# AE-HYU/monte_carlo_localization

Hardware: AMD Instinct MI355X
Metric: MCL updates/sec (particle*beam/s) (higher is better)
Workload: dtype f64; 1 GPU; 4194304 particles/GPU x 1081 beams, Spielberg_map (2000x2000 @ 0.05796), initial cloud N((0.0, 0.0, 0.0),(0.5 m,0.5 m,0.4 rad)) (tracking regime), action (0.05, 0.0, 0.01), stock sensor/motion params, multinomial resampling, Philox seed 42; the timed updates follow 5 warm-up updates (the particle set has resampled to motion-noise width); particles_total=4194304, beams=1081, parallelism=single GPU

## Files before the change

### include/mcl_hip_engine.h

```cpp
#ifndef MCL_HIP_ENGINE_H
#define MCL_HIP_ENGINE_H

#include <stddef.h>
#include <stdint.h>

#ifdef __cplusplus
extern "C" {
#endif

#define MCL_ABI_VERSION 1

typedef struct mcl_engine mcl_engine_t;

typedef enum {
    MCL_OK = 0,
    MCL_ERR_INVALID_ARG = -1,
    MCL_ERR_NOT_READY = -2,
    MCL_ERR_HIP = -3,
    MCL_ERR_NO_DEVICE = -4,
    MCL_ERR_UNSUPPORTED = -5,
    MCL_ERR_PEER = -6,
    MCL_ERR_TIMEOUT = -7
} mcl_status;

// ... 231 lines not shown
    int32_t reserved;
} mcl_recovery_config_t;
void mcl_default_recovery_config(mcl_recovery_config_t *c);
int mcl_set_recovery(mcl_engine_t *h, const mcl_recovery_config_t *c);
int mcl_get_recovery_state(mcl_engine_t *h, double state[3], int64_t *injected_last);
int mcl_set_recovery_state(mcl_engine_t *h, const double state[2]);
int mcl_host_recovery_step(const mcl_recovery_config_t *c, const double in[2], int32_t reset, double max_logw, double sum_w,
                           double denom, int32_t n_beams, double out[2], double *p_next);
int mcl_set_recovery_proposal(mcl_engine_t *h, int32_t n_components, const double *means ,
                              const double *covs , const double *weights );
int mcl_get_recovery_proposal(const mcl_engine_t *h, int32_t *n_components, uint64_t *thresholds, double *factors);
int mcl_host_recovery_proposal(int32_t n_components, const double *means, const double *covs, const double *weights,
                               uint64_t *thresholds, double *factors);

typedef struct {
    double z_hit, z_rand;
    double sigma_hit_m;
    double max_occ_dist_m;
    int32_t reserved[2];
} mcl_likelihood_field_config_t;
void mcl_default_likelihood_field_config(mcl_likelihood_field_config_t *c);
int mcl_set_likelihood_field(mcl_engine_t *h, const mcl_likelihood_field_config_t *c);
int mcl_get_likelihood_field(mcl_engine_t *h, uint16_t *out, size_t n);
int mcl_get_likelihood_table(mcl_engine_t *h, float *out, size_t n, int32_t *K);
int mcl_host_likelihood_field(const int8_t *data, uint32_t width, uint32_t height, float resolution,
                              const mcl_likelihood_field_config_t *c, uint16_t *out, size_t n);
int mcl_host_likelihood_table(const mcl_config_t *cfg, const mcl_likelihood_field_config_t *c, float resolution, float *out,
                              size_t n, int32_t *K);

typedef enum { MCL_MOTION_REFERENCE = 0, MCL_MOTION_DIFF = 1, MCL_MOTION_OMNI = 2 } mcl_motion_model;
typedef struct {
    int32_t model;
    int32_t reserved;
    double alpha1, alpha2, alpha3, alpha4, alpha5;
    double floor_trans_m, floor_rot_rad;
} mcl_motion_config_t;
void mcl_default_motion_config(mcl_motion_config_t *c);
int mcl_set_motion_model(mcl_engine_t *h, const mcl_motion_config_t *c);
int mcl_get_motion_model(const mcl_engine_t *h, mcl_motion_config_t *out);
int mcl_host_motion_scalars(const mcl_motion_config_t *c, const double action[3], double out[8]);
int mcl_host_motion_sample(const mcl_motion_config_t *c, const double action[3], const double *xyz_colmajor,
                           const double *normals_nx3, int64_t n, double *out_colmajor);
int mcl_init_particles_gaussian(mcl_engine_t *h, const double mean[3], const double cov[9], int64_t n,
                                int64_t first_global_index, int64_t n_total);
int mcl_host_gaussian_factor(const double cov[9], double L[6]);
int mcl_init_particles_mixture(mcl_engine_t *h, int32_t n_components, const double *means, const double *covs, const int64_t *counts,
                               int64_t n, int64_t first_global_index, int64_t n_total);

int mcl_host_sensor_table(const mcl_config_t *cfg, int32_t max_range_px, double *out, size_t n);
int mcl_host_skip_field(const int8_t *data, uint32_t width, uint32_t height, uint8_t *out, size_t n);
int mcl_host_skip_field_dir(const int8_t *data, uint32_t width, uint32_t height, int32_t quadrant, uint8_t *out, size_t n);
#define MCL_WEDGES 16
int mcl_host_skip_field_wedge(const int8_t *data, uint32_t width, uint32_t height, int32_t wedge, uint8_t *out, size_t n);
int mcl_host_sweep_global_layout(uint32_t width, uint32_t height, int32_t max_range_px, int64_t out[6]);

typedef enum {
    MCL_BUF_X = 0, MCL_BUF_Y = 1, MCL_BUF_THETA = 2,
    MCL_BUF_QWEIGHT = 3,
    MCL_BUF_LOGW = 4,
    MCL_BUF_SCALARS = 5
} mcl_buffer_id;
int mcl_device_ptr(mcl_engine_t *h, int32_t which, void **dev_ptr);
int mcl_export_state(mcl_engine_t *h, double *d_x, double *d_y, double *d_theta, uint64_t *d_q);
int mcl_get_scalars(mcl_engine_t *h, double out[8]);
int mcl_get_host_scalars(const mcl_engine_t *h, double out[8]);
int mcl_stage_propagate(mcl_engine_t *h, const double *d_px, const double *d_py, const double *d_pth,
                        const uint64_t *d_cdf, int64_t n_parents, uint64_t q_total,
                        int64_t child_first, int64_t n_children_total,
                        const double action[3], const float *obs, int32_t n_beams);
int mcl_stage_resample(mcl_engine_t *h, const double *d_px, const double *d_py, const double *d_pth,
                       const uint64_t *d_cdf, int64_t n_parents, uint64_t q_total,
                       int64_t child_first, int64_t n_children_total, const double action[3]);
int mcl_export_records(mcl_engine_t *h, void *d_records);
int mcl_stage_resample_records(mcl_engine_t *h, const void *d_records, const uint64_t *d_cdf, int64_t n_parents,
                               uint64_t q_total, int64_t child_first, int64_t n_children_total, const double action[3]);
int mcl_stage_distinct_parents(mcl_engine_t *h, const int32_t *d_parent, int64_t n_children, int64_t n_total,
                               int64_t *d_distinct, int32_t *d_slot, int64_t *count);
int mcl_export_records_at(mcl_engine_t *h, const int64_t *d_index, int64_t count, void *d_out);
int mcl_stage_resample_indices(mcl_engine_t *h, const uint64_t *d_cdf, int64_t n_parents, uint64_t q_total, int64_t child_first,
                               int64_t n_children_total, int32_t *d_parent_idx);
int mcl_stage_motion_records(mcl_engine_t *h, const void *d_records, int64_t n_records, const int32_t *d_record_of_child,
                             int64_t child_first, int64_t n_children_total, const double action[3]);
int mcl_compact_chunk_bytes(int64_t chunk_entries, int64_t *bytes);
int mcl_export_compact(mcl_engine_t *h, void *d_chunk, int64_t chunk_entries);
int mcl_stage_resample_compact(mcl_engine_t *h, const void *d_chunks, int32_t n_shards, int64_t chunk_entries, const int64_t *counts,
                               const uint64_t *totals, int64_t n_per_shard, int32_t self_shard, int64_t child_first, int64_t n_children_total,
                               const double action[3]);
int mcl_stage_rays(mcl_engine_t *h, const float *obs, int32_t n_beams);
int mcl_set_reserved_cus(mcl_engine_t *h, int32_t n_cus);
int mcl_stage_weights(mcl_engine_t *h, double global_max_logw);
int mcl_stage_finish(mcl_engine_t *h, const double global_sums[5]);
int mcl_stage_keep(mcl_engine_t *h, int64_t child_first, int64_t n_children_total, const double action[3]);
int mcl_stream_wait_external(mcl_engine_t *h, void *stream);
int mcl_external_wait_stream(mcl_engine_t *h, void *stream);
int mcl_export_compact_async(mcl_engine_t *h, void *d_chunk, int64_t chunk_entries);
int mcl_stage_resample_compact_async(mcl_engine_t *h, const void *d_chunks, int32_t n_shards, int64_t chunk_entries, const int64_t *counts,
                                     const uint64_t *totals, int64_t n_per_shard, int32_t self_shard, int64_t child_first,
                                     int64_t n_children_total, const double action[3]);
int mcl_stage_rays_async(mcl_engine_t *h, const float *obs, int32_t n_beams, double *d_local_max);
int mcl_stage_weights_async(mcl_engine_t *h, const double *d_global_max, double *d_vec, int32_t n_shards, int32_t self_shard);
int mcl_stage_complete(mcl_engine_t *h, const double global_sums[5], int32_t *redo);
int mcl_comm_available(const char **why);
int mcl_comm_unique_id(unsigned char id[128]);
int mcl_comm_create(mcl_engine_t *h, const unsigned char id[128], int32_t n_ranks, int32_t rank);
int mcl_comm_selftest(mcl_engine_t *h);
int mcl_comm_destroy(mcl_engine_t *h);
// ... 36 lines not shown
```

### monte_carlo_localization_amd/csrc/mcl_engine.hip

```cpp
#include "../../include/mcl_hip_engine.h"

#include <hip/hip_runtime.h>
#include <hip/hip_ext.h>
#include <rocprim/device/device_radix_sort.hpp>

#include <algorithm>
#include <chrono>
#include <cmath>
#include <cstdio>
#include <cstring>
#include <string>
#include <vector>

#include "mcl_engine_internal.h"
#include "mcl_kernels.h"
#include "mcl_host_math.h"
#include "mcl_lfield.h"

static_assert(MCL_WEDGES == mcl::kWedges || MCL_KWEDGES != 16, "include/mcl_hip_engine.h and csrc/mcl_wedge.h disagree");

using namespace mcl_host;

namespace {

// ... 921 lines not shown
    h->grid_host.assign(data, data + (size_t)width * height);
    h->map_epoch++;
    h->Wp = h->W + 1; h->Hp = h->H + 1; h->Wps = (h->Wp + 7) & ~7;
    h->tw_cells = 568;
    { const int S = h->env_qside > 0 ? h->env_qside : 280; h->qside = (S - (P + 2) - 3 >= 32) ? S : 0; }
    h->sweep_global = h->env_sweep_global || !mcl::sweep_window_fits(P);
    h->distg_why_not = nullptr;
    const bool want_wedges = h->qside > 0 || h->sweep_global;
    build_sensor_table(h->cfg, P, h->table);
    const int tw = P + 1;
    std::vector<float> L((size_t)tw * tw);
    const double inv_squash = 1.0 / h->cfg.squash_factor;
    for (int r = 0; r < tw; ++r)
        for (int d = 0; d < tw; ++d) L[(size_t)r * tw + d] = (float)(std::log(h->table[(size_t)d * tw + r]) * inv_squash);
    std::vector<uint8_t> dist;
    build_distance_field(data, h->W, h->H, h->Wp, h->Hp, h->Wps, dist);
    h->have_map = false;
    h->d_grid.drop(); h->d_dist.drop(); h->d_dist4.drop(); h->d_L.drop(); h->d_table.drop();
    for (int q = 0; q < 4; ++q) h->d_distq[q].drop();
    MCL_TRY(h->d_grid.reserve(h, (size_t)h->W * h->H));
    MCL_TRY(h->d_dist.reserve(h, dist.size()));
    MCL_TRY(h->d_L.reserve(h, L.size()));
    MCL_TRY(h->d_table.reserve(h, h->table.size()));
    HIPCHK(h, hipMemcpy(h->d_grid, data, (size_t)h->W * h->H, hipMemcpyHostToDevice));
    HIPCHK(h, hipMemcpy(h->d_dist, dist.data(), dist.size(), hipMemcpyHostToDevice));
    {
        std::vector<uint8_t> d4(dist.size() / 2);
        for (size_t k = 0; k < d4.size(); ++k)
            d4[k] = (uint8_t)(std::min<int>(dist[2 * k], 15) | (std::min<int>(dist[2 * k + 1], 15) << 4));
        MCL_TRY(h->d_dist4.reserve(h, d4.size()));
        HIPCHK(h, hipMemcpy(h->d_dist4, d4.data(), d4.size(), hipMemcpyHostToDevice));
    }
    if (want_wedges) {
        static const int qsx[4] = {1, -1, -1, 1}, qsy[4] = {1, 1, -1, -1};
        std::vector<uint8_t> dq;
        for (int q = 0; q < 4; ++q) {
            build_directional_field(data, h->W, h->H, h->Wp, h->Hp, h->Wps, qsx[q], qsy[q], dq);
            MCL_TRY(h->d_distq[q].reserve(h, dq.size()));
            HIPCHK(h, hipMemcpy(h->d_distq[q], dq.data(), dq.size(), hipMemcpyHostToDevice));
        }
    }
    h->d_distw.drop(); h->d_distg.drop();
    if (want_wedges) {
        const size_t fsz = (size_t)h->Hp * h->Wps, ncell = (size_t)h->Hp * h->Wp;
        DevBuf<int32_t> d_nxt, d_prv;
        DevBuf<mcl::WedgeRow> d_rows;
        std::vector<mcl::WedgeRow> rows(2 * mcl::kWedgeR + 1);
        MCL_TRY(h->d_distw.reserve(h, fsz * mcl::kWedges));
        HIPCHK(h, hipMemsetAsync(h->d_distw, 0, fsz * mcl::kWedges, h->stream));
        MCL_TRY(d_nxt.reserve(h, ncell));
        MCL_TRY(d_prv.reserve(h, ncell));
        MCL_TRY(d_rows.reserve(h, rows.size()));
        hipLaunchKernelGGL(mcl::k_row_tables, dim3((h->Hp + 63) / 64), dim3(64), 0, h->stream, h->d_dist, h->Wp, h->Hp, h->Wps, d_nxt, d_prv);
        int rc_w = MCL_OK;
        for (int k = 0; k < mcl::kWedges && rc_w == MCL_OK; ++k) {
            mcl::wedge_rows(k, rows.data());
            if (hipMemcpyAsync(d_rows, rows.data(), rows.size() * sizeof(mcl::WedgeRow), hipMemcpyHostToDevice, h->stream) != hipSuccess ||
                hipStreamSynchronize(h->stream) != hipSuccess) { rc_w = MCL_ERR_HIP; break; }
            hipLaunchKernelGGL(mcl::k_wedge_field, dim3((h->Wp + 255) / 256, h->Hp), dim3(256), 0, h->stream, d_nxt, d_prv, h->Wp, h->Hp, h->Wps,
                               d_rows, h->d_distw + (size_t)k * fsz);
            if (hipStreamSynchronize(h->stream) != hipSuccess) rc_w = MCL_ERR_HIP;
        }
        if (rc_w != MCL_OK) return fail(h, rc_w, "building the wedge fields failed");
        if (h->sweep_global) {
            const mcl::SweepGlobalLayout gl = mcl::sweep_global_layout(h->Wp, h->Hp, P);
            if (!gl.ok) {
                h->distg_why_not = "k_rays_sweep's global-field form needs the sixteen ringed fields (with their tails) in less than 2^32 bytes and rows / pitch below 2^24: this map is too large for it";
            } else {
                h->distg_pitch = gl.pitch;
                h->distg_stride = gl.stride;
                MCL_TRY(h->d_distg.reserve(h, gl.alloc));
                HIPCHK(h, hipMemsetAsync(h->d_distg, 0xFF, gl.alloc, h->stream));
                for (int k = 0; k < mcl::kWedges; ++k) {
                    const int q = k >> mcl::kWedgeShift;
                    hipLaunchKernelGGL(mcl::k_ring_field, dim3((h->distg_pitch + 255) / 256, h->Hp + 4), dim3(256), 0, h->stream, h->d_distw + (size_t)k * fsz,
                                       h->Wp, h->Hp, h->Wps, h->distg_pitch, (q == 0 || q == 3) ? 1 : 0, (q == 0 || q == 1) ? 1 : 0,
                                       h->d_distg + (size_t)k * h->distg_stride);
                }
                HIPCHK(h, hipGetLastError());
                HIPCHK(h, hipStreamSynchronize(h->stream));
            }
        }
    }
    HIPCHK(h, hipMemcpy(h->d_L, L.data(), L.size() * sizeof(float), hipMemcpyHostToDevice));
    HIPCHK(h, hipMemcpy(h->d_table, h->table.data(), h->table.size() * sizeof(double), hipMemcpyHostToDevice));
    h->d_Lt.drop(); h->d_Ltd.drop(); h->ltd_ready = false;
    {
        std::vector<uint32_t> fr;
        for (size_t i = 0; i < (size_t)h->W * h->H; ++i)
            if (data[i] == 0) fr.push_back((uint32_t)i);
        h->d_free.drop();
        h->n_free = fr.size();
        if (h->n_free) {
            MCL_TRY(h->d_free.reserve(h, fr.size()));
            HIPCHK(h, hipMemcpy(h->d_free, fr.data(), fr.size() * sizeof(uint32_t), hipMemcpyHostToDevice));
        }
    }
    h->have_map = true;
    if (h->kld_on) {
        h->kld_nx = kld_nx; h->kld_ny = kld_ny; h->kld_bits = kld_bits;
        const int rc = kld_alloc(h);
        if (rc) { h->have_map = false; return rc; }
    }
    h->lf_K = -1;
    if (h->lf_on) {
        const int rc = lf_build(h);
        if (rc) { h->have_map = false; return rc; }
    }
    return MCL_OK;
}

int mcl_get_max_range_px(const mcl_engine_t *h, int32_t *out)
// ... 1683 lines not shown
```

### monte_carlo_localization_amd/csrc/mcl_host_math.hip

```cpp
#include "mcl_host_math.h"

#include <algorithm>
#include <cmath>
#include <cstring>

#include "mcl_motion.h"
#include "mcl_refine_core.h"
#include "mcl_wedge.h"

namespace mcl_host {

const char *bad_sensor_fields(const mcl_config_t &c)
{
    const double z[4] = {c.z_hit, c.z_short, c.z_max, c.z_rand};
    for (double v : z)
        if (!std::isfinite(v) || v < 0.0) return "bad config (z_hit, z_short, z_max and z_rand must be finite and >= 0)";
    if (z[0] == 0.0 && z[1] == 0.0 && z[2] == 0.0 && z[3] == 0.0) return "bad config (z_hit, z_short, z_max and z_rand are all 0)";
    if (!std::isfinite(c.sigma_hit) || !(c.sigma_hit > 0.0)) return "bad config (sigma_hit must be finite and > 0)";
    return nullptr;
}

void build_sensor_table(const mcl_config_t &c, int P, std::vector<double> &t)
{
    const int tw = P + 1;
// ... 652 lines not shown
        if (thresholds) thresholds[c] = c == M - 1 ? (1ull << 53) : (uint64_t)std::floor((s / total) * 9007199254740992.0);
        if (factors) {
            double *f = factors + 9 * (size_t)c;
            for (int k = 0; k < 3; ++k) f[k] = means[3 * (size_t)c + k];
            (void)gaussian_factor(covs + 9 * (size_t)c, f + 3);
        }
    }
    return std::string();
}

}

using namespace mcl_host;

extern "C" {

void mcl_default_config(mcl_config_t *c)
{
    if (!c) return;
    std::memset(c, 0, sizeof(*c));
    c->max_particles = 2000;
    c->device = 0;
    c->seed = 0;
    c->max_range_m = 12.0;
    c->z_hit = 0.80; c->z_short = 0.01; c->z_max = 0.07; c->z_rand = 0.12; c->sigma_hit = 8.0;
    c->squash_factor = 2.2;
    c->motion_dispersion_x = 0.05; c->motion_dispersion_y = 0.025; c->motion_dispersion_theta = 0.25;
    c->resample_mode = MCL_RESAMPLE_MULTINOMIAL;
    c->weight_mode = MCL_WEIGHT_LOG;
    c->ray_kernel = MCL_RAYS_AUTO;
}

int mcl_host_sensor_table(const mcl_config_t *cfg, int32_t P, double *out, size_t n)
{
    if (!cfg || !out || P < 1 || n != (size_t)(P + 1) * (P + 1) || bad_sensor_fields(*cfg)) return MCL_ERR_INVALID_ARG;
    std::vector<double> t;
    build_sensor_table(*cfg, P, t);
    std::memcpy(out, t.data(), n * sizeof(double));
    return MCL_OK;
}

int mcl_host_skip_field_dir(const int8_t *data, uint32_t width, uint32_t height, int32_t quadrant, uint8_t *out, size_t n)
{
    if (!data || !out || width == 0 || height == 0 || quadrant < 0 || quadrant > 3 || n != (size_t)(width + 1) * (height + 1))
        return MCL_ERR_INVALID_ARG;
    static const int qsx[4] = {1, -1, -1, 1}, qsy[4] = {1, 1, -1, -1};
    const int Wp = (int)width + 1, Hp = (int)height + 1, Wps = (Wp + 7) & ~7;
    std::vector<uint8_t> d;
    build_directional_field(data, (int)width, (int)height, Wp, Hp, Wps, qsx[quadrant], qsy[quadrant], d);
    for (int y = 0; y < Hp; ++y) std::memcpy(out + (size_t)y * Wp, d.data() + (size_t)y * Wps, Wp);
    return MCL_OK;
}

int mcl_host_skip_field_wedge(const int8_t *data, uint32_t width, uint32_t height, int32_t wedge, uint8_t *out, size_t n)
{
    if (!data || !out || width == 0 || height == 0 || wedge < 0 || wedge >= mcl::kWedges || n != (size_t)(width + 1) * (height + 1))
        return MCL_ERR_INVALID_ARG;
    const int W = (int)width, H = (int)height, Wp = W + 1, Hp = H + 1;
    std::vector<int32_t> nxt((size_t)Wp * Hp), prv((size_t)Wp * Hp);
    for (int y = 0; y < Hp; ++y) {
        auto stop = [&](int x) { return data[(size_t)std::max(y - 1, 0) * W + std::max(x - 1, 0)] > 50; };
        int last = -1;
        for (int x = 0; x < Wp; ++x) { if (stop(x)) last = x; prv[(size_t)y * Wp + x] = last; }
        int next = Wp;
        for (int x = Wp - 1; x >= 0; --x) { if (stop(x)) next = x; nxt[(size_t)y * Wp + x] = next; }
    }
    std::vector<mcl::WedgeRow> rows(2 * mcl::kWedgeR + 1);
    mcl::wedge_rows(wedge, rows.data());
    for (int y = 0; y < Hp; ++y)
        for (int x = 0; x < Wp; ++x) out[(size_t)y * Wp + x] = (uint8_t)mcl::wedge_skip_cell(nxt.data(), prv.data(), Wp, Hp, x, y, rows.data());
    return MCL_OK;
}

int mcl_host_skip_field(const int8_t *data, uint32_t width, uint32_t height, uint8_t *out, size_t n)
{
    if (!data || !out || width == 0 || height == 0 || n != (size_t)(width + 1) * (height + 1)) return MCL_ERR_INVALID_ARG;
    const int Wp = (int)width + 1, Hp = (int)height + 1, Wps = (Wp + 7) & ~7;
    std::vector<uint8_t> d;
    build_distance_field(data, (int)width, (int)height, Wp, Hp, Wps, d);
    for (int y = 0; y < Hp; ++y) std::memcpy(out + (size_t)y * Wp, d.data() + (size_t)y * Wps, Wp);
    return MCL_OK;
}

int mcl_host_sweep_global_layout(uint32_t width, uint32_t height, int32_t max_range_px, int64_t out[6])
{
    if (!out || width == 0 || height == 0 || max_range_px < 1) return MCL_ERR_INVALID_ARG;
    const int Wp = (int)width + 1, Hp = (int)height + 1;
    const mcl::SweepGlobalLayout g = mcl::sweep_global_layout(Wp, Hp, max_range_px);
    out[0] = g.ok ? 1 : 0; out[1] = g.pitch; out[2] = g.rows; out[3] = (int64_t)g.stride; out[4] = (int64_t)g.alloc;
    out[5] = (int64_t)mcl::sweep_global_max_offset(g, Wp, Hp, max_range_px, mcl::kWedges - 1);
    return MCL_OK;
}

void mcl_default_kld_config(mcl_kld_config_t *k)
{
    if (!k) return;
    *k = mcl_kld_config_t{};
    k->min_particles = 256; k->max_particles = 4194304;
    k->err = 0.01; k->z = 2.326;
    k->bin_x_m = 0.5; k->bin_y_m = 0.5;
    k->n_theta_bins = 36; k->round_to = 256; k->shrink_permille = 800;
}

int mcl_host_kld_bins(const double *x, const double *y, const double *th, int64_t n, uint32_t width, uint32_t height,
                      float resolution, double origin_x, double origin_y, const mcl_kld_config_t *k, int64_t *bins)
{
    if (!k || !bins || n < 0 || (n > 0 && (!x || !y || !th)) || width == 0 || height == 0 || !(resolution > 0.0f) ||
        !std::isfinite(resolution) || kld_invalid(k, 0))
        return MCL_ERR_INVALID_ARG;
    int64_t nx = 0, ny = 0;
    uint64_t nbits = 0;
    if (!kld_grid(k, width, height, resolution, nx, ny, nbits)) return MCL_ERR_INVALID_ARG;
    const mcl::KldArgs a = kld_args_of(k, nx, ny, origin_x, origin_y);
    std::vector<uint32_t> b((size_t)n);
    for (int64_t i = 0; i < n; ++i) b[(size_t)i] = mcl::kld_bin(a, x[i], y[i], th[i]);
    std::sort(b.begin(), b.end());
    *bins = (int64_t)(std::unique(b.begin(), b.end()) - b.begin());
    return MCL_OK;
}

int mcl_host_kld_target(const mcl_kld_config_t *k, int64_t bins, int64_t n_current, int64_t *n_next)
{
    if (!k || !n_next || n_current < 0 || n_current >= MCL_MAX_TOTAL_PARTICLES || kld_invalid(k, 0)) return MCL_ERR_INVALID_ARG;
// ... 342 lines not shown
```

### monte_carlo_localization_amd/csrc/mcl_kernels.h

```cpp
#pragma once
#include "mcl_types.h"
#include <type_traits>
#include "mcl_ray_core.h"
#include "mcl_device_math.h"
#include "mcl_wedge.h"
#include "mcl_motion.h"

namespace mcl {

constexpr int kRedBlocks = 1024;
constexpr int kRedThreads = 256;
__device__ __forceinline__ void final_sums_of(const double *__restrict__ part, int nb, double *__restrict__ scalars, double (*sm)[7]);


__device__ __forceinline__ uint64_t wave_incl_scan_u64(uint64_t v, int lane)
{
#pragma unroll
    for (int o = 1; o < 64; o <<= 1) {
        uint64_t t = (uint64_t)__shfl_up((long long)v, o, 64);
        if (lane >= o) v += t;
    }
    return v;
}

// ... 1091 lines not shown
        cnt_l2 = wave_sum_u64(cnt_l2);
        if (lane == 0) {
            if (cnt_exact) atomicAdd(&a.counters[0], cnt_exact);
            if (cnt_off) atomicAdd(&a.counters[1], cnt_off);
            if (cnt_probe) atomicAdd(&a.counters[2], cnt_probe);
            if (cnt_l2) atomicAdd(&a.counters[3], cnt_l2);
        }
    }
}

constexpr int kQLdsBase = 16;

__device__ __forceinline__ void quad_ranges(short4 qr, int q, int B, int &ja, int &jb, int &ja2)
{
    const int st1 = qr.x & 0x3FFF, st2 = qr.y, st3 = qr.z, st4 = qr.w, q0 = ((int)qr.x >> 14) & 3;
    const int r_idx = (q - q0) & 3;
    ja = r_idx == 0 ? 0 : (r_idx == 1 ? st1 : (r_idx == 2 ? st2 : st3));
    jb = r_idx == 0 ? st1 : (r_idx == 1 ? st2 : (r_idx == 2 ? st3 : st4));
    ja2 = r_idx == 0 ? st4 : B;
}


__global__ __launch_bounds__(256) void k_ring_field(const uint8_t *__restrict__ src, int Wp, int Hp, int Wps, int pitch, int sxp, int syp,
                                                   uint8_t *__restrict__ dst)
{
    const int x = blockIdx.x * blockDim.x + threadIdx.x, y = blockIdx.y;
    if (x >= pitch) return;
    const int mx = x - 2, my = y - 2;
    uint8_t v = 0xFF;
    if (mx >= 0 && mx < Wp && my >= 0 && my < Hp) v = src[(size_t)(syp ? my : Hp - 1 - my) * Wps + (sxp ? mx : Wp - 1 - mx)];
    dst[(size_t)y * pitch + x] = v;
}

__global__ void k_row_tables(const uint8_t *__restrict__ dist, int Wp, int Hp, int Wps, int32_t *__restrict__ nxt, int32_t *__restrict__ prv)
{
    const int y = blockIdx.x * blockDim.x + threadIdx.x;
    if (y >= Hp) return;
    const uint8_t *row = dist + (size_t)y * Wps;
    int last = -1;
    for (int x = 0; x < Wp; ++x) { if (row[x] == 0) last = x; prv[(size_t)y * Wp + x] = last; }
    int next = Wp;
    for (int x = Wp - 1; x >= 0; --x) { if (row[x] == 0) next = x; nxt[(size_t)y * Wp + x] = next; }
}

__global__ __launch_bounds__(256) void k_wedge_field(const int32_t *__restrict__ nxt, const int32_t *__restrict__ prv, int Wp, int Hp, int Wps,
                                                    const WedgeRow *__restrict__ rows, uint8_t *__restrict__ out)
{
    const int x = blockIdx.x * blockDim.x + threadIdx.x, y = blockIdx.y;
    if (x >= Wp || y >= Hp) return;
    const int v = wedge_skip_cell(nxt, prv, Wp, Hp, x, y, rows);
    out[(size_t)y * Wps + x] = (uint8_t)(v == 0 ? 255 : (v > 127 ? 127 : v));
}

#ifndef MCL_SORT_KEY_LOG2
#define MCL_SORT_KEY_LOG2 22
#endif
constexpr int kSortKeyLog2 = MCL_SORT_KEY_LOG2;
constexpr uint32_t kSortKeySpace = 1u << kSortKeyLog2;
#ifndef MCL_SORT_MAX_SUB
#define MCL_SORT_MAX_SUB 1
#endif
constexpr int kSortXcds = 8;
constexpr uint32_t kSortBuckets = kSortKeySpace * kSortXcds;
constexpr int kHistTile = 4096;

__device__ __forceinline__ int cell_of(double g, int hi)
{
    int c = (g > -1.0) ? ((g < 1e9) ? (int)floor(g) + 1 : hi) : 0;
    return c < 0 ? 0 : (c > hi ? hi : c);
}

__global__ void k_bbox_init(int *__restrict__ bbox, int play)
{
    const int i = threadIdx.x;
    if (i < 7) bbox[i] = i < 2 ? 0x7fffffff : (i < 4 ? (int)0x80000000 : (i == 6 ? play : 0));
}

__global__ __launch_bounds__(256) void k_cell_bbox(const double4 *__restrict__ pc, int64_t n, int stride, int Wp, int Hp, int *__restrict__ bbox,
                                                  int *__restrict__ tilemark = nullptr, int ntx_abs = 0)
{
    int x0 = 0x7fffffff, y0 = 0x7fffffff, x1 = -1, y1 = -1;
    const int64_t ns = (n + stride - 1) / stride;
    for (int64_t k = (int64_t)blockIdx.x * blockDim.x + threadIdx.x; k < ns; k += (int64_t)gridDim.x * blockDim.x) {
        const double4 c = pc[k * stride];
        const int cx = cell_of(c.z * kSortSub, Wp * kSortSub - 1), cy = cell_of(c.w * kSortSub, Hp * kSortSub - 1);
        x0 = min(x0, cx); y0 = min(y0, cy); x1 = max(x1, cx); y1 = max(y1, cy);
        if (tilemark) tilemark[(cy >> 5) * ntx_abs + (cx >> 5)] = 1;
    }
#pragma unroll
    for (int o = 32; o > 0; o >>= 1) {
        x0 = min(x0, __shfl_xor(x0, o, 64)); y0 = min(y0, __shfl_xor(y0, o, 64));
        x1 = max(x1, __shfl_xor(x1, o, 64)); y1 = max(y1, __shfl_xor(y1, o, 64));
    }
    __shared__ int red[4][4];
    const int w = threadIdx.x >> 6;
    if ((threadIdx.x & 63) == 0) { red[w][0] = x0; red[w][1] = y0; red[w][2] = x1; red[w][3] = y1; }
    __syncthreads();
    if (threadIdx.x == 0) {
        for (int k = 1; k < 4; ++k) { x0 = min(x0, red[k][0]); y0 = min(y0, red[k][1]); x1 = max(x1, red[k][2]); y1 = max(y1, red[k][3]); }
        if (x1 >= 0) { atomicMin(&bbox[0], x0); atomicMin(&bbox[1], y0); atomicMax(&bbox[2], x1); atomicMax(&bbox[3], y1); }
    }
}

constexpr int kSortMaxTiles = 8192;
__global__ __launch_bounds__(1024) void k_tile_compact(int *__restrict__ bbox, int *__restrict__ tilemark, int *__restrict__ tilemap, int ntiles_abs)
{
// ... 876 lines not shown
```

### monte_carlo_localization_amd/csrc/mcl_wedge.h

```cpp
#pragma once
#include <cmath>
#include <cstdint>

#ifdef __HIPCC__
#define MCL_HD __host__ __device__
#else
#define MCL_HD
#endif

namespace mcl {

#ifndef MCL_KWEDGES
#define MCL_KWEDGES 16
#endif
constexpr int kWedges = MCL_KWEDGES;
constexpr int kWedgeShift = kWedges == 8 ? 1 : kWedges == 16 ? 2 : kWedges == 32 ? 3 : 4;
static_assert(kWedges == (4 << kWedgeShift), "kWedges must be 8, 16, 32 or 64");
constexpr int kWedgeR = 255;

struct WedgeRow { int16_t xa, xb; };

inline void wedge_rows(int k, WedgeRow *rows)
{
    const double two_pi = 6.283185307179586476925286766559;
// ... 5 lines not shown
    const int sx = (q == 0 || q == 3) ? 1 : -1, sy = (q == 0 || q == 1) ? 1 : -1;
    for (int oy = -kWedgeR; oy <= kWedgeR; ++oy) {
        int xa = 1, xb = 0;
        bool any = false;
        for (int ox = -kWedgeR; ox <= kWedgeR; ++ox) {
            const bool in = sx * ox >= 0 && sy * oy >= 0 && (n1x * ox + n1y * oy + e1 > 1e-9) && (n2x * ox + n2y * oy + e2 > 1e-9);
            if (in) { if (!any) { xa = ox; any = true; } xb = ox; }
        }
        rows[oy + kWedgeR].xa = (int16_t)xa;
        rows[oy + kWedgeR].xb = (int16_t)xb;
    }
}

MCL_HD inline int wedge_skip_cell(const int32_t *nxt, const int32_t *prv, int Wp, int Hp, int x, int y, const WedgeRow *rows)
{
    if (nxt[(size_t)y * Wp + x] == x) return 0;
    int64_t best = (int64_t)1 << 40;
    for (int d = 0; d <= kWedgeR; ++d) {
        const int64_t gy = d > 1 ? d - 1 : 0;
        if (gy * gy >= best) break;
        for (int sgn = (d == 0 ? 1 : -1); sgn <= 1; sgn += 2) {
            const int oy = sgn * d;
            const WedgeRow r = rows[oy + kWedgeR];
            if (r.xa > r.xb) continue;
            const int yy = y + oy, lo = x + r.xa, hi = x + r.xb;
            const bool row_in = yy >= 0 && yy < Hp;
            int ox = 1 << 20;
            if (r.xa <= 0 && r.xb >= 0) {
                const int xr = row_in ? nxt[(size_t)yy * Wp + x] : x;
                const int xl = row_in ? prv[(size_t)yy * Wp + x] : x;
                if (xr <= hi) ox = xr - x;
                if (xl >= lo && x - xl < ox) ox = x - xl;
            } else if (r.xa > 0) {
                const int xr = (!row_in || lo >= Wp) ? lo : nxt[(size_t)yy * Wp + lo];
                if (xr <= hi) ox = xr - x;
            } else {
                const int xl = (!row_in || hi < 0) ? hi : prv[(size_t)yy * Wp + hi];
                if (xl >= lo) ox = x - xl;
            }
            if (ox < (1 << 20)) {
                const int64_t gx = ox > 1 ? ox - 1 : 0;
                const int64_t g2 = gx * gx + gy * gy;
                if (g2 < best) best = g2;
            }
        }
    }
    if (best >= (int64_t)254 * 254) return 255;
    int64_t rt = (int64_t)sqrt((double)best);
    while (rt * rt > best) --rt;
    while ((rt + 1) * (rt + 1) <= best) ++rt;
    return (int)(rt + 1);
}

struct SweepGlobalLayout { bool ok; int pitch; int rows; size_t stride, alloc; };
inline SweepGlobalLayout sweep_global_layout(int Wp, int Hp, int P)
{
    SweepGlobalLayout g{};
    g.pitch = (Wp + 4 + 63) & ~63;
    const int tail = P + 2 + (P + 4 + g.pitch - 1) / g.pitch;
    g.rows = Hp + 4 + tail;
    g.stride = (size_t)g.rows * (size_t)g.pitch;
    g.alloc = g.stride * (size_t)kWedges;
    g.ok = g.alloc < ((size_t)1 << 32) && g.rows + P < (1 << 24) && g.pitch < (1 << 24) && P >= 1;
    return g;
}
inline size_t sweep_global_max_offset(const SweepGlobalLayout &g, int Wp, int Hp, int P, int k)
{
    return (size_t)k * g.stride + (size_t)(Hp + 4 + P) * (size_t)g.pitch + (size_t)(Wp + 4 + P);
}

}
```

### monte_carlo_localization_amd/engine.py

```python
from __future__ import annotations

import ctypes as C
import os

import numpy as np

_HERE = os.path.dirname(os.path.abspath(__file__))
LIB_PATH = os.environ.get("MCL_LIB") or os.path.join(_HERE, "libmcl_hip_engine.so")

MCL_OK = 0
MCL_ERR_INVALID_ARG = -1
MCL_ERR_NOT_READY = -2
MCL_ERR_PEER = -6
MCL_ERR_TIMEOUT = -7
RESAMPLE_MULTINOMIAL, RESAMPLE_SYSTEMATIC = 0, 1
WEIGHT_LOG, WEIGHT_PRODUCT = 0, 1
RAYS_AUTO, RAYS_MARCH, RAYS_SKIP, RAYS_QUAD, RAYS_CELL, RAYS_SWEEP = 0, 1, 2, 3, 4, 5
BUF_X, BUF_Y, BUF_THETA, BUF_QWEIGHT, BUF_LOGW, BUF_SCALARS = range(6)

EXPORTS = [
    "mcl_abi_version", "mcl_default_config", "mcl_create", "mcl_destroy", "mcl_last_error", "mcl_set_map",
    "mcl_get_max_range_px", "mcl_get_sensor_table", "mcl_set_beam_angles", "mcl_set_particles",
    "mcl_get_particles", "mcl_get_weights", "mcl_sample_particles", "mcl_particle_mean", "mcl_update",
    "mcl_sensor_update", "mcl_expected_pose", "mcl_get_stage_timings", "mcl_get_resample_indices",
    "mcl_get_ray_steps", "mcl_get_log_weights", "mcl_get_counters", "mcl_get_ray_kernel_ms", "mcl_device_ptr",
    "mcl_stage_propagate", "mcl_stage_weights", "mcl_stage_finish", "mcl_scan_weights", "mcl_export_state",
    "mcl_get_scalars", "mcl_host_sensor_table", "mcl_host_skip_field", "mcl_init_particles_pose", "mcl_init_global",
    "mcl_update_scan", "mcl_get_ray_kernel_id", "mcl_host_skip_field_dir", "mcl_host_skip_field_wedge", "mcl_export_records", "mcl_get_effective_sample_size", "mcl_get_host_scalars", "mcl_stage_resample_records", "mcl_stage_resample", "mcl_stage_rays",
    "mcl_set_reserved_cus", "mcl_stage_resample_indices", "mcl_stage_motion_records", "mcl_stage_distinct_parents", "mcl_export_records_at",
    "mcl_group_create", "mcl_group_destroy", "mcl_group_last_error", "mcl_group_size", "mcl_group_engine", "mcl_group_set_map",
    "mcl_group_set_beam_angles", "mcl_group_set_particles", "mcl_group_init_particles_pose", "mcl_group_init_global",
    "mcl_group_update", "mcl_group_expected_pose", "mcl_group_get_particles", "mcl_group_get_weights",
    "mcl_group_get_resample_indices", "mcl_group_get_stage_timings", "mcl_group_exchange_bytes",
    "mcl_set_debug_count_probes", "mcl_set_particles_shard", "mcl_get_compact_list", "mcl_compact_chunk_bytes", "mcl_export_compact",
    "mcl_stage_resample_compact", "mcl_group_exchanged_lists", "mcl_get_ray_steps16", "mcl_get_planned_ray_kernel",
    "mcl_stream_wait_external", "mcl_external_wait_stream", "mcl_export_compact_async", "mcl_stage_resample_compact_async",
    "mcl_stage_rays_async", "mcl_stage_weights_async", "mcl_stage_complete", "mcl_stage_keep",
    "mcl_comm_available", "mcl_comm_unique_id", "mcl_comm_create", "mcl_comm_destroy", "mcl_comm_update", "mcl_comm_stats", "mcl_comm_set_lists", "mcl_comm_get_vector", "mcl_comm_last_exchange", "mcl_comm_selftest",
    "mcl_host_sweep_global_layout", "mcl_get_ray_kernel_variant",
    "mcl_default_kld_config", "mcl_set_kld", "mcl_get_particle_count", "mcl_get_kld_state", "mcl_host_kld_bins", "mcl_host_kld_target",
    "mcl_default_cluster_config", "mcl_pose_clusters", "mcl_get_cluster_labels",
    "mcl_query_scans", "mcl_score_poses", "mcl_get_query_counters",
    "mcl_default_search_config", "mcl_global_search", "mcl_get_search_scores", "mcl_get_search_bytes", "mcl_host_search_lattice",
    "mcl_host_search_headings", "mcl_init_particles_mixture",
    "mcl_global_search_sequence", "mcl_host_search_sequence_offsets", "mcl_host_relative_poses",
    "mcl_default_search_stream_config", "mcl_global_search_streamed", "mcl_host_search_slabs",
    "mcl_global_search_beam", "mcl_host_search_beam_grid", "mcl_get_search_beam_table",
    "mcl_default_search_prune_config", "mcl_global_search_pruned", "mcl_get_search_bounds", "mcl_host_search_blocks", "mcl_host_lf_pool",
    "mcl_host_search_bound_table", "mcl_host_search_prune_next",
    "mcl_default_refine_config", "mcl_refine_poses", "mcl_refine_poses_beam", "mcl_get_refine_scores", "mcl_get_refine_bytes", "mcl_host_refine_window",
    "mcl_host_refine_reduce",
    "mcl_default_recovery_config", "mcl_set_recovery", "mcl_get_recovery_state", "mcl_set_recovery_state", "mcl_host_recovery_step",
    "mcl_set_recovery_proposal", "mcl_get_recovery_proposal", "mcl_host_recovery_proposal",
    "mcl_default_likelihood_field_config", "mcl_set_likelihood_field", "mcl_get_likelihood_field", "mcl_get_likelihood_table",
    "mcl_host_likelihood_field", "mcl_host_likelihood_table",
    "mcl_default_motion_config", "mcl_set_motion_model", "mcl_get_motion_model", "mcl_host_motion_scalars", "mcl_host_motion_sample",
    "mcl_init_particles_gaussian", "mcl_host_gaussian_factor", "mcl_group_set_motion_model", "mcl_group_init_particles_gaussian",
]
MOTION_REFERENCE, MOTION_DIFF, MOTION_OMNI = 0, 1, 2
MOTION_MODELS = {"reference": MOTION_REFERENCE, "diff": MOTION_DIFF, "omni": MOTION_OMNI}


class Config(C.Structure):
    _fields_ = [
        ("max_particles", C.c_int64), ("device", C.c_int32), ("seed", C.c_uint64), ("max_range_m", C.c_double),
        ("z_hit", C.c_double), ("z_short", C.c_double), ("z_max", C.c_double), ("z_rand", C.c_double),
        ("sigma_hit", C.c_double), ("squash_factor", C.c_double), ("motion_dispersion_x", C.c_double),
        ("motion_dispersion_y", C.c_double), ("motion_dispersion_theta", C.c_double), ("resample_mode", C.c_int32),
        ("weight_mode", C.c_int32), ("ray_kernel", C.c_int32), ("keep_ray_steps", C.c_int32),
        ("debug_force_exact", C.c_int32), ("debug_count_probes", C.c_int32), ("rays_per_lane", C.c_int32),
        ("resample_neff_permille", C.c_int32), ("graph_mode", C.c_int32), ("reserved", C.c_int32 * 3),
    ]


class KldConfig(C.Structure):
    _fields_ = [
        ("min_particles", C.c_int64), ("max_particles", C.c_int64), ("err", C.c_double), ("z", C.c_double),
        ("bin_x_m", C.c_double), ("bin_y_m", C.c_double), ("n_theta_bins", C.c_int32), ("round_to", C.c_int32),
        ("shrink_permille", C.c_int32), ("reserved", C.c_int32),
    ]


class RecoveryConfig(C.Structure):
    _fields_ = [("alpha_slow", C.c_double), ("alpha_fast", C.c_double), ("per_beam", C.c_int32), ("reserved", C.c_int32)]


class LikelihoodFieldConfig(C.Structure):
    _fields_ = [("z_hit", C.c_double), ("z_rand", C.c_double), ("sigma_hit_m", C.c_double), ("max_occ_dist_m", C.c_double),
                ("reserved", C.c_int32 * 2)]


class MotionConfig(C.Structure):
# ... 577 lines not shown
    if rc != MCL_OK:
        raise EngineError(f"mcl_host_kld_bins rc={rc}", rc)
    return out.value


def host_kld_target(kld: KldConfig, bins: int, n_current: int) -> int:
    out = C.c_int64()
    rc = load_library().mcl_host_kld_target(C.byref(kld), int(bins), int(n_current), C.byref(out))
    if rc != MCL_OK:
        raise EngineError(f"mcl_host_kld_target rc={rc}", rc)
    return out.value


def _p(a):
    return None if a is None else a.ctypes.data_as(C.c_void_p)


def _c(a, dt):
    return None if a is None else np.ascontiguousarray(a, dtype=dt)


def host_sensor_table(P: int, cfg: Config | None = None) -> np.ndarray:
    cfg = cfg or default_config()
    out = np.empty((P + 1) * (P + 1), np.float64)
    rc = load_library().mcl_host_sensor_table(C.byref(cfg), C.c_int32(P), _p(out), C.c_size_t(out.size))
    if rc != MCL_OK:
        raise EngineError(f"mcl_host_sensor_table rc={rc}")
    return out.reshape(P + 1, P + 1)


def host_skip_field(grid) -> np.ndarray:
    g = _c(grid, np.int8)
    H, W = g.shape
    out = np.empty((H + 1, W + 1), np.uint8)
    rc = load_library().mcl_host_skip_field(_p(g), C.c_uint32(W), C.c_uint32(H), _p(out), C.c_size_t(out.size))
    if rc != MCL_OK:
        raise EngineError(f"mcl_host_skip_field rc={rc}")
    return out


WEDGES = 16


def host_skip_field_wedge(grid, wedge: int) -> np.ndarray:
    g = _c(grid, np.int8)
    H, W = g.shape
    out = np.empty((H + 1, W + 1), np.uint8)
    rc = load_library().mcl_host_skip_field_wedge(_p(g), C.c_uint32(W), C.c_uint32(H), C.c_int32(wedge), _p(out), C.c_size_t(out.size))
    if rc != MCL_OK:
        raise EngineError(f"mcl_host_skip_field_wedge rc={rc}")
    return out


def host_skip_field_dir(grid, quadrant: int) -> np.ndarray:
    g = _c(grid, np.int8)
    H, W = g.shape
    out = np.empty((H + 1, W + 1), np.uint8)
    rc = load_library().mcl_host_skip_field_dir(_p(g), C.c_uint32(W), C.c_uint32(H), C.c_int32(quadrant), _p(out), C.c_size_t(out.size))
    if rc != MCL_OK:
        raise EngineError(f"mcl_host_skip_field_dir rc={rc}")
    return out


class Engine:

    def __init__(self, cfg: Config | None = None, **over):
        self.cfg = cfg if cfg is not None else default_config(**over)
        if cfg is not None:
            for k, v in over.items():
                setattr(self.cfg, k, v)
        self.lib = load_library(legacy=int(self.cfg.ray_kernel) in (RAYS_QUAD, RAYS_CELL))
        h = C.c_void_p()
        rc = self.lib.mcl_create(C.byref(self.cfg), C.byref(h))
        if rc != MCL_OK:
            raise EngineError(f"mcl_create rc={rc}: {self.lib.mcl_last_error(None).decode()}")
        self._h = h
        self.n = 0
        self.n_beams = 0

    def close(self):
        if getattr(self, "_h", None):
            if not getattr(self, "_borrowed", False):
                self.lib.mcl_destroy(self._h)
            self._h = None

    def __del__(self):
        try:
            self.close()
        except Exception:
            pass

    def _chk(self, rc, what):
        if rc != MCL_OK:
            raise EngineError(f"{what} rc={rc}: {self.lib.mcl_last_error(self._h).decode()}", rc)

    def set_map(self, grid, resolution, origin_x, origin_y):
        g = _c(grid, np.int8)
        H, W = g.shape
        self._chk(self.lib.mcl_set_map(self._h, _p(g), C.c_uint32(W), C.c_uint32(H), C.c_float(np.float32(resolution)),
                                       C.c_double(origin_x), C.c_double(origin_y)), "mcl_set_map")
        self.map_shape = (H, W)
        self.map_resolution = float(np.float32(resolution))

    @property
    def max_range_px(self) -> int:
        v = C.c_int32()
# ... 784 lines not shown
```

Baseline: 877.0 billion particle*beam/s.

## Use tighter cone-aware skip distances for wedge empty-space fields

```diff
diff --git a/include/mcl_hip_engine.h b/include/mcl_hip_engine.h
--- a/include/mcl_hip_engine.h
+++ b/include/mcl_hip_engine.h
@@ -307,6 +307,8 @@
 int mcl_host_skip_field_dir(const int8_t *data, uint32_t width, uint32_t height, int32_t quadrant, uint8_t *out, size_t n);
 #define MCL_WEDGES 16
 int mcl_host_skip_field_wedge(const int8_t *data, uint32_t width, uint32_t height, int32_t wedge, uint8_t *out, size_t n);
+int mcl_host_skip_field_wedge_tight(const int8_t *data, uint32_t width, uint32_t height, int32_t wedge, uint8_t *out, size_t n);
+int mcl_host_wedge_tight_table(int32_t wedge, int32_t *values, uint8_t *reachable, size_t n);
 int mcl_host_sweep_global_layout(uint32_t width, uint32_t height, int32_t max_range_px, int64_t out[6]);
 
 typedef enum {
diff --git a/monte_carlo_localization_amd/csrc/mcl_engine.hip b/monte_carlo_localization_amd/csrc/mcl_engine.hip
--- a/monte_carlo_localization_amd/csrc/mcl_engine.hip
+++ b/monte_carlo_localization_amd/csrc/mcl_engine.hip
@@ -997,12 +997,18 @@
         MCL_TRY(d_prv.reserve(h, ncell));
         MCL_TRY(d_rows.reserve(h, rows.size()));
         hipLaunchKernelGGL(mcl::k_row_tables, dim3((h->Hp + 63) / 64), dim3(64), 0, h->stream, h->d_dist, h->Wp, h->Hp, h->Wps, d_nxt, d_prv);
+        const char *env_metric = getenv("MCL_WEDGE_METRIC");
+        const bool tight = !(env_metric && atoi(env_metric) == 0);
         int rc_w = MCL_OK;
         for (int k = 0; k < mcl::kWedges && rc_w == MCL_OK; ++k) {
             mcl::wedge_rows(k, rows.data());
             if (hipMemcpyAsync(d_rows, rows.data(), rows.size() * sizeof(mcl::WedgeRow), hipMemcpyHostToDevice, h->stream) != hipSuccess ||
                 hipStreamSynchronize(h->stream) != hipSuccess) { rc_w = MCL_ERR_HIP; break; }
-            hipLaunchKernelGGL(mcl::k_wedge_field, dim3((h->Wp + 255) / 256, h->Hp), dim3(256), 0, h->stream, d_nxt, d_prv, h->Wp, h->Hp, h->Wps,
+            if (tight)
+                hipLaunchKernelGGL(mcl::k_wedge_field_tight, dim3((h->Wp + 255) / 256, h->Hp), dim3(256), 0, h->stream, d_nxt, d_prv, h->Wp, h->Hp, h->Wps,
+                                   d_rows, mcl::wedge_cone(k), h->d_distw + (size_t)k * fsz);
+            else
+                hipLaunchKernelGGL(mcl::k_wedge_field, dim3((h->Wp + 255) / 256, h->Hp), dim3(256), 0, h->stream, d_nxt, d_prv, h->Wp, h->Hp, h->Wps,
                                d_rows, h->d_distw + (size_t)k * fsz);
             if (hipStreamSynchronize(h->stream) != hipSuccess) rc_w = MCL_ERR_HIP;
         }
diff --git a/monte_carlo_localization_amd/csrc/mcl_host_math.hip b/monte_carlo_localization_amd/csrc/mcl_host_math.hip
--- a/monte_carlo_localization_amd/csrc/mcl_host_math.hip
+++ b/monte_carlo_localization_amd/csrc/mcl_host_math.hip
@@ -728,7 +728,36 @@
     return MCL_OK;
 }
 
+static int host_wedge_field(const int8_t *data, uint32_t width, uint32_t height, int32_t wedge, uint8_t *out, size_t n, bool tight);
+
 int mcl_host_skip_field_wedge(const int8_t *data, uint32_t width, uint32_t height, int32_t wedge, uint8_t *out, size_t n)
+{
+    return host_wedge_field(data, width, height, wedge, out, n, false);
+}
+
+int mcl_host_skip_field_wedge_tight(const int8_t *data, uint32_t width, uint32_t height, int32_t wedge, uint8_t *out, size_t n)
+{
+    return host_wedge_field(data, width, height, wedge, out, n, true);
+}
+
+int mcl_host_wedge_tight_table(int32_t wedge, int32_t *values, uint8_t *reachable, size_t n)
+{
+    const int S = 2 * mcl::kWedgeR + 1;
+    if (wedge < 0 || wedge >= mcl::kWedges || !values || !reachable || n != (size_t)S * S) return MCL_ERR_INVALID_ARG;
+    std::vector<mcl::WedgeRow> rows(S);
+    mcl::wedge_rows(wedge, rows.data());
+    const mcl::WedgeCone cone = mcl::wedge_cone(wedge);
+    for (int oy = -mcl::kWedgeR; oy <= mcl::kWedgeR; ++oy)
+        for (int ox = -mcl::kWedgeR; ox <= mcl::kWedgeR; ++ox) {
+            const size_t i = (size_t)(oy + mcl::kWedgeR) * S + (size_t)(ox + mcl::kWedgeR);
+            const mcl::WedgeRow r = rows[oy + mcl::kWedgeR];
+            reachable[i] = (ox >= r.xa && ox <= r.xb) ? 1 : 0;
+            values[i] = mcl::wedge_tight_value(cone, ox, oy);
+        }
+    return MCL_OK;
+}
+
+static int host_wedge_field(const int8_t *data, uint32_t width, uint32_t height, int32_t wedge, uint8_t *out, size_t n, bool tight)
 {
     if (!data || !out || width == 0 || height == 0 || wedge < 0 || wedge >= mcl::kWedges || n != (size_t)(width + 1) * (height + 1))
         return MCL_ERR_INVALID_ARG;
@@ -743,8 +772,11 @@
     }
     std::vector<mcl::WedgeRow> rows(2 * mcl::kWedgeR + 1);
     mcl::wedge_rows(wedge, rows.data());
+    const mcl::WedgeCone cone = mcl::wedge_cone(wedge);
     for (int y = 0; y < Hp; ++y)
-        for (int x = 0; x < Wp; ++x) out[(size_t)y * Wp + x] = (uint8_t)mcl::wedge_skip_cell(nxt.data(), prv.data(), Wp, Hp, x, y, rows.data());
+        for (int x = 0; x < Wp; ++x)
+            out[(size_t)y * Wp + x] = (uint8_t)(tight ? mcl::wedge_skip_cell_tight(nxt.data(), prv.data(), Wp, Hp, x, y, rows.data(), cone)
+                                                      : mcl::wedge_skip_cell(nxt.data(), prv.data(), Wp, Hp, x, y, rows.data()));
     return MCL_OK;
 }
 
diff --git a/monte_carlo_localization_amd/csrc/mcl_kernels.h b/monte_carlo_localization_amd/csrc/mcl_kernels.h
--- a/monte_carlo_localization_amd/csrc/mcl_kernels.h
+++ b/monte_carlo_localization_amd/csrc/mcl_kernels.h
@@ -1167,6 +1167,15 @@
     out[(size_t)y * Wps + x] = (uint8_t)(v == 0 ? 255 : (v > 127 ? 127 : v));
 }
 
+__global__ __launch_bounds__(256) void k_wedge_field_tight(const int32_t *__restrict__ nxt, const int32_t *__restrict__ prv, int Wp, int Hp, int Wps,
+                                                          const WedgeRow *__restrict__ rows, WedgeCone cone, uint8_t *__restrict__ out)
+{
+    const int x = blockIdx.x * blockDim.x + threadIdx.x, y = blockIdx.y;
+    if (x >= Wp || y >= Hp) return;
+    const int v = wedge_skip_cell_tight(nxt, prv, Wp, Hp, x, y, rows, cone);
+    out[(size_t)y * Wps + x] = (uint8_t)(v == 0 ? 255 : (v > 127 ? 127 : v));
+}
+
 #ifndef MCL_SORT_KEY_LOG2
 #define MCL_SORT_KEY_LOG2 22
 #endif
diff --git a/monte_carlo_localization_amd/csrc/mcl_wedge.h b/monte_carlo_localization_amd/csrc/mcl_wedge.h
--- a/monte_carlo_localization_amd/csrc/mcl_wedge.h
+++ b/monte_carlo_localization_amd/csrc/mcl_wedge.h
@@ -81,6 +81,101 @@
     return (int)(rt + 1);
 }
 
+constexpr double kWedgeWiden = 1e-7;
+constexpr double kWedgeSlack = 1e-6;
+
+struct WedgeCone {
+    double ax, ay, bx, by;
+    double iax, iay, ibx, iby;
+};
+
+inline WedgeCone wedge_cone(int k)
+{
+    const double two_pi = 6.283185307179586476925286766559;
+    const double a0 = two_pi * k / kWedges - kWedgeWiden, a1 = two_pi * (k + 1) / kWedges + kWedgeWiden;
+    WedgeCone w;
+    w.ax = std::cos(a0); w.ay = std::sin(a0); w.bx = std::cos(a1); w.by = std::sin(a1);
+    w.iax = 1.0 / w.ax; w.iay = 1.0 / w.ay; w.ibx = 1.0 / w.bx; w.iby = 1.0 / w.by;
+    return w;
+}
+
+MCL_HD inline double wedge_ray_entry(double ex, double ey, double iex, double iey, double lx, double hx, double ly, double hy)
+{
+    double t0 = 0.0, t1 = 1e30;
+    if (ex == 0.0) { if (lx > 0.0 || hx < 0.0) return -1.0; }
+    else { const double p = lx * iex, q = hx * iex; t0 = fmax(t0, fmin(p, q)); t1 = fmin(t1, fmax(p, q)); }
+    if (ey == 0.0) { if (ly > 0.0 || hy < 0.0) return -1.0; }
+    else { const double p = ly * iey, q = hy * iey; t0 = fmax(t0, fmin(p, q)); t1 = fmin(t1, fmax(p, q)); }
+    return t0 <= t1 ? t0 : -1.0;
+}
+
+MCL_HD inline int wedge_isqrt(int64_t v)
+{
+    int64_t rt = (int64_t)sqrt((double)v);
+    while (rt * rt > v) --rt;
+    while ((rt + 1) * (rt + 1) <= v) ++rt;
+    return (int)rt;
+}
+
+MCL_HD inline int wedge_tight_value(const WedgeCone &w, int ox, int oy)
+{
+    const int ax = ox < 0 ? -ox : ox, ay = oy < 0 ? -oy : oy;
+    const int gx = ax > 1 ? ax - 1 : 0, gy = ay > 1 ? ay - 1 : 0;
+    const int base = wedge_isqrt((int64_t)gx * gx + (int64_t)gy * gy) + 1;
+    if (gx == 0 && gy == 0) return base;
+    const double nx = ox < 0 ? -(double)gx : (double)gx, ny = oy < 0 ? -(double)gy : (double)gy;
+    if (w.ax * ny - w.ay * nx >= 0.0 && nx * w.by - ny * w.bx >= 0.0) return base;
+    const double lx = ox - 1.0, hx = ox + 1.0, ly = oy - 1.0, hy = oy + 1.0;
+    const double ta = wedge_ray_entry(w.ax, w.ay, w.iax, w.iay, lx, hx, ly, hy);
+    const double tb = wedge_ray_entry(w.bx, w.by, w.ibx, w.iby, lx, hx, ly, hy);
+    double D = -1.0;
+    if (ta >= 0.0) D = ta;
+    if (tb >= 0.0 && (D < 0.0 || tb < D)) D = tb;
+    if (D < 0.0) return base;
+    const int v = (int)floor(D - kWedgeSlack) + 1;
+    return v > base ? v : base;
+}
+
+MCL_HD inline int wedge_skip_cell_tight(const int32_t *nxt, const int32_t *prv, int Wp, int Hp, int x, int y, const WedgeRow *rows,
+                                        const WedgeCone &w)
+{
+    if (nxt[(size_t)y * Wp + x] == x) return 0;
+    int best = 255;
+    for (int d = 0; d <= kWedgeR; ++d) {
+        if (d >= best) break;
+        for (int sgn = (d == 0 ? 1 : -1); sgn <= 1; sgn += 2) {
+            const int oy = sgn * d;
+            const WedgeRow r = rows[oy + kWedgeR];
+            if (r.xa > r.xb) continue;
+            const int yy = y + oy, lo = x + r.xa, hi = x + r.xb;
+            const bool row_in = yy >= 0 && yy < Hp;
+            int oxr = 1 << 20, oxl = 1 << 20;
+            if (r.xa <= 0 && r.xb >= 0) {
+                const int xr = row_in ? nxt[(size_t)yy * Wp + x] : x;
+                const int xl = row_in ? prv[(size_t)yy * Wp + x] : x;
+                if (xr <= hi) oxr = xr - x;
+                if (xl >= lo) oxl = x - xl;
+            } else if (r.xa > 0) {
+                const int xr = (!row_in || lo >= Wp) ? lo : nxt[(size_t)yy * Wp + lo];
+                if (xr <= hi) oxr = xr - x;
+            } else {
+                const int xl = (!row_in || hi < 0) ? hi : prv[(size_t)yy * Wp + hi];
+                if (xl >= lo) oxl = x - xl;
+            }
+            const int64_t gy = d > 1 ? d - 1 : 0, lim = (int64_t)(best - 1) * (best - 1);
+            if (oxr < (1 << 20)) {
+                const int64_t gx = oxr > 1 ? oxr - 1 : 0;
+                if (gx * gx + gy * gy < lim) { const int v = wedge_tight_value(w, oxr, oy); if (v < best) best = v; }
+            }
+            if (oxl < (1 << 20) && oxl != 0) {
+                const int64_t gx = oxl > 1 ? oxl - 1 : 0;
+                if (gx * gx + gy * gy < lim) { const int v = wedge_tight_value(w, -oxl, oy); if (v < best) best = v; }
+            }
+        }
+    }
+    return best;
+}
+
 struct SweepGlobalLayout { bool ok; int pitch; int rows; size_t stride, alloc; };
 inline SweepGlobalLayout sweep_global_layout(int Wp, int Hp, int P)
 {
diff --git a/monte_carlo_localization_amd/engine.py b/monte_carlo_localization_amd/engine.py
--- a/monte_carlo_localization_amd/engine.py
+++ b/monte_carlo_localization_amd/engine.py
@@ -37,7 +37,7 @@
     "mcl_stream_wait_external", "mcl_external_wait_stream", "mcl_export_compact_async", "mcl_stage_resample_compact_async",
     "mcl_stage_rays_async", "mcl_stage_weights_async", "mcl_stage_complete", "mcl_stage_keep",
     "mcl_comm_available", "mcl_comm_unique_id", "mcl_comm_create", "mcl_comm_destroy", "mcl_comm_update", "mcl_comm_stats", "mcl_comm_set_lists", "mcl_comm_get_vector", "mcl_comm_last_exchange", "mcl_comm_selftest",
-    "mcl_host_sweep_global_layout", "mcl_get_ray_kernel_variant",
+    "mcl_host_sweep_global_layout", "mcl_get_ray_kernel_variant", "mcl_host_skip_field_wedge_tight", "mcl_host_wedge_tight_table",
     "mcl_default_kld_config", "mcl_set_kld", "mcl_get_particle_count", "mcl_get_kld_state", "mcl_host_kld_bins", "mcl_host_kld_target",
     "mcl_default_cluster_config", "mcl_pose_clusters", "mcl_get_cluster_labels",
     "mcl_query_scans", "mcl_score_poses", "mcl_get_query_counters",
@@ -721,6 +721,28 @@
     return out
 
 
+def host_skip_field_wedge_tight(grid, wedge: int) -> np.ndarray:
+    g = _c(grid, np.int8)
+    H, W = g.shape
+    out = np.empty((H + 1, W + 1), np.uint8)
+    rc = load_library().mcl_host_skip_field_wedge_tight(_p(g), C.c_uint32(W), C.c_uint32(H), C.c_int32(wedge), _p(out), C.c_size_t(out.size))
+    if rc != MCL_OK:
+        raise EngineError(f"mcl_host_skip_field_wedge_tight rc={rc}")
+    return out
+
+
+WEDGE_R = 255
+
+
+def host_wedge_tight_table(wedge: int):
+    S = 2 * WEDGE_R + 1
+    val, reach = np.empty((S, S), np.int32), np.empty((S, S), np.uint8)
+    rc = load_library().mcl_host_wedge_tight_table(C.c_int32(wedge), _p(val), _p(reach), C.c_size_t(val.size))
+    if rc != MCL_OK:
+        raise EngineError(f"mcl_host_wedge_tight_table rc={rc}")
+    return val, reach.astype(bool)
+
+
 def host_skip_field_dir(grid, quadrant: int) -> np.ndarray:
     g = _c(grid, np.int8)
     H, W = g.shape
```

Measured after the change: 890.3 billion particle*beam/s, median of 6. 1.5% higher.
